# krea-ai/realtime-video

Measured on AMD Instinct MI355X. Metric: frames/sec at 832x480, 4-step 14B T2V (per-step DiT latency in config), higher is better.
Workload: dtype bf16

## Files before the change

### realtime_video_amd/csrc/gemm8.hip

```cpp
#include <atomic>
#include <mutex>
#include <type_traits>

#include "gemm_core.h"
#include "gemm_split.h"
#include "rtv_internal.h"

#ifndef RTV_G8_MFMA16
#define RTV_G8_MFMA16 1
#endif

namespace rtv {

namespace g8 {
constexpr int BM = 256, BN = 256, BK = 64;
constexpr int HALF_BYTES = 128 * BK * 2;
constexpr int A_OFF = 0;
constexpr int W_OFF = 6 * HALF_BYTES;
constexpr int LDS_BYTES = 10 * HALF_BYTES;
constexpr int THREADS = 512;
__device__ __forceinline__ int swz(int row, int chunk) { return chunk ^ ((row >> 1) & 7); }
}

#ifdef RTV_GEMM_TIMELINE
__device__ unsigned long long* g_timeline = nullptr;
#endif

__device__ __forceinline__ void g8_tile_mn(int tiles_m, int tiles_n, int tile_id, int* mt, int* nt) {
#if RTV_G8_BALANCED_GROUPS
  const int ngrp = (tiles_m + 7) >> 3;
  const int gq = tiles_m / ngrp, gr = tiles_m - gq * ngrp;
  const int big = (gq + 1) * tiles_n;
  int first_m, gm, in_group;
  if (tile_id < gr * big) {
    const int group = tile_id / big;
    gm = gq + 1;
    first_m = group * gm;
    in_group = tile_id - group * big;
  } else {
    const int t = tile_id - gr * big, sm = gq * tiles_n, group = t / sm;
    gm = gq;
    first_m = gr * (gq + 1) + group * gq;
    in_group = t - group * sm;
  }
#else
  constexpr int GROUP_M = 8;
  const int per_group = GROUP_M * tiles_n;
  const int group = tile_id / per_group;
  const int first_m = group * GROUP_M;
  const int gm = min(tiles_m - first_m, GROUP_M);
  const int in_group = tile_id - group * per_group;
#endif
  *mt = first_m + in_group % gm;
  *nt = in_group / gm;
}

template <bool F16>
__device__ __forceinline__ void gemm8m_body(const GemmParams& p, const SplitArgs& sp, int m0, int n0, int tile_id, int seg, int unit,
                                            int kt_begin, int kt_end, bool is_split);

template <bool F16, bool SKIP_IDLE>
__global__ __launch_bounds__(g8::THREADS, 2) void gemm8_kernel(GemmParams p, SplitArgs sp) {
  using namespace g8;
  int bid0 = blockIdx.x;
  if (sp.pair_units) {
    if (bid0 < sp.pair_pad) {
      if (bid0 >= sp.pair_units) return;
#pragma unroll 1
      for (int j = 0; j < 2; ++j) {
        const int tn = 2 * bid0 + j;
        if (tn >= p.tiles_n) break;
        if (j) __syncthreads();
        gemm8m_body<F16>(p, sp, sp.pair_m0, tn * BN, 0, 0, -1, 0, p.K / BK, false);
      }
      return;
    }
    bid0 -= sp.pair_pad;
  }
  if (sp.half_tail) {
    const int nhu = 2 * sp.tail_tiles;
    if (sp.split_first) bid0 = bid0 < nhu ? sp.first_unit + bid0 : bid0 - nhu;
    if (bid0 >= sp.first_unit) {
      const int v = xcd_remap(bid0 - sp.first_unit, nhu);
      const int tile_id = sp.first_unit + (v >> 1);
      int mt, nt;
      g8_tile_mn(p.tiles_m, p.tiles_n, tile_id, &mt, &nt);
      const int m0h = mt * BM + (v & 1) * 128;
      if (m0h >= p.M) return;
      gemm8m_body<F16>(p, sp, m0h, nt * BN, tile_id, 0, -1, 0, p.K / BK, false);
      return;
    }
    sp.S = 1;
    sp.split_first = 0;
  }
#ifdef RTV_GEMM_TIMELINE
  const unsigned long long tl_t0 = __builtin_amdgcn_s_memrealtime();
  const unsigned long long tl_c0 = __builtin_amdgcn_s_memtime();
  unsigned long long tl_t1 = 0;
#endif
  [[maybe_unused]] typedef TileCfg<256, 256, 64, 2, 4> Cfg;
  extern __shared__ __attribute__((aligned(16))) char smem[];

  const int tid = threadIdx.x;
  const int lane = tid & 63;
  const int wave = __builtin_amdgcn_readfirstlane(tid >> 6);
  const int wr = wave >> 2, wc = wave & 3;
  [[maybe_unused]] const int l31 = lane & 31, g = lane >> 5;

  const int nk_total = p.K / BK;
  int tile_id, seg, unit, kt_begin, kt_end;
  const bool is_split = split_unit_of_block(sp, bid0, nk_total, &tile_id, &unit, &seg, &kt_begin, &kt_end);
  int mt_, nt_;
  g8_tile_mn(p.tiles_m, p.tiles_n, tile_id, &mt_, &nt_);
  const int m0 = mt_ * BM;
  const int n0 = nt_ * BN;
  uint32_t src_off[4][2];
  {
    const int rsub = lane >> 3, cpos = lane & 7;
#pragma unroll
    for (int j = 0; j < 2; ++j) {
      const int row = j * 64 + wave * 8 + rsub;
      const int ch = swz(row, cpos) * 8;
#pragma unroll
      for (int h = 0; h < 2; ++h) {
        const int gm_row = min(m0 + h * 128 + row, p.M - 1);
        const int gn_row = min(n0 + h * 128 + row, p.N - 1);
        src_off[h][j] = ((uint32_t)gm_row * (uint32_t)p.lda + ch) * 2u;
        src_off[2 + h][j] = ((uint32_t)gn_row * (uint32_t)p.ldw + ch) * 2u;
      }
    }
  }
  __amdgpu_buffer_rsrc_t rsrcA = __builtin_amdgcn_make_buffer_rsrc((void*)p.A, 0, 0x7fffffff, 0x00020000);
  __amdgpu_buffer_rsrc_t rsrcW = __builtin_amdgcn_make_buffer_rsrc((void*)p.W, 0, 0x7fffffff, 0x00020000);
  auto stage_piece = [&](int kt, int a3, int h, int j, auto chk) {
    if (decltype(chk)::value && kt >= kt_end) return;
    const int slot = h < 2 ? A_OFF + (a3 * 2 + h) * HALF_BYTES : W_OFF + ((kt & 1) * 2 + (h - 2)) * HALF_BYTES;
    __builtin_amdgcn_raw_ptr_buffer_load_lds(h < 2 ? rsrcA : rsrcW, (RTV_LDS void*)(smem + slot + (j * 64 + wave * 8) * 128), 16,
                                             src_off[h][j], (unsigned)kt * (BK * 2), 0, 0);
  };

  const int b_row0 = (wc & 1) * 64;
#if RTV_G8_MFMA16
  const int l15 = lane & 15, q4 = lane >> 4;
  u32x4 af[4][2];
  u32x4 bfr[4][2];
  auto read_a = [&](int a3, int mq) {
    const char* s = smem + A_OFF + (a3 * 2 + wr) * HALF_BYTES;
#pragma unroll
    for (int mb = 0; mb < 4; ++mb) {
      const int row = mq * 64 + mb * 16 + l15;
#pragma unroll
      for (int ks = 0; ks < 2; ++ks) af[mb][ks] = *(const u32x4*)(s + row * 128 + (swz(row, ks * 4 + q4) << 4));
    }
  };
  auto read_w = [&](int wb) {
    const char* s = smem + W_OFF + (wb * 2 + (wc >> 1)) * HALF_BYTES;
#pragma unroll
    for (int nb = 0; nb < 4; ++nb) {
      const int row = b_row0 + nb * 16 + l15;
#pragma unroll
      for (int ks = 0; ks < 2; ++ks) bfr[nb][ks] = *(const u32x4*)(s + row * 128 + (swz(row, ks * 4 + q4) << 4));
    }
  };

  f32x4 acc[8][4];
#pragma unroll
  for (int mi = 0; mi < 8; ++mi)
#pragma unroll
    for (int ni = 0; ni < 4; ++ni)
#pragma unroll
      for (int r = 0; r < 4; ++r) acc[mi][ni][r] = 0.f;
#else
  u32x4 af[2][4];
  u32x4 bfr[2][4];
  auto read_a = [&](int a3, int mq) {
    const char* s = smem + A_OFF + (a3 * 2 + wr) * HALF_BYTES;
#pragma unroll
    for (int mb = 0; mb < 2; ++mb) {
      const int row = mq * 64 + mb * 32 + l31;
#pragma unroll
      for (int ks = 0; ks < 4; ++ks) af[mb][ks] = *(const u32x4*)(s + row * 128 + (swz(row, ks * 2 + g) << 4));
    }
  };
  auto read_w = [&](int wb) {
    const char* s = smem + W_OFF + (wb * 2 + (wc >> 1)) * HALF_BYTES;
#pragma unroll
    for (int nq = 0; nq < 2; ++nq) {
      const int row = b_row0 + nq * 32 + l31;
#pragma unroll
      for (int ks = 0; ks < 4; ++ks) bfr[nq][ks] = *(const u32x4*)(s + row * 128 + (swz(row, ks * 2 + g) << 4));
    }
  };

  f32x16 acc[4][2];
#pragma unroll
  for (int mi = 0; mi < 4; ++mi)
#pragma unroll
    for (int ni = 0; ni < 2; ++ni)
#pragma unroll
      for (int r = 0; r < 16; ++r) acc[mi][ni][r] = 0.f;
#endif

#define G8_FENCE() __builtin_amdgcn_sched_barrier(0)
#if RTV_G8_MFMA16
#define G8_STORE_LDS(...) store_tile_lds16<F16>(__VA_ARGS__)
#define G8_STORE_DIRECT(CFG, ...) store_tile16<F16>(__VA_ARGS__)
#else
#define G8_STORE_LDS(...) store_tile_lds<F16>(__VA_ARGS__)
#define G8_STORE_DIRECT(CFG, ...) store_tile<F16, CFG>(__VA_ARGS__)
#endif
#define G8_BARRIER()                  \
  do {                                \
    G8_FENCE();                       \
    __builtin_amdgcn_s_barrier();     \
    G8_FENCE();                       \
  } while (0)
#define G8_LDS_DONE()                                   \
  do {                                                  \
    asm volatile("s_waitcnt lgkmcnt(0)" ::: "memory");  \
    G8_FENCE();                                         \
  } while (0)

  const bool idle_rows = SKIP_IDLE && m0 + wr * 128 >= p.M;
  auto mma_half = [&](int mq, int st_kt, int st_a3, int h0, auto chk) {
    __builtin_amdgcn_s_setprio(1);
    int n = 0;
#if RTV_G8_MFMA16
#pragma unroll
    for (int ks = 0; ks < 2; ++ks)
#pragma unroll
      for (int nb = 0; nb < 4; ++nb)
#pragma unroll
        for (int mb = 0; mb < 4; ++mb) {
          acc[mq * 4 + mb][nb] = Mfma16<F16>::run(bfr[nb][ks], af[mb][ks], acc[mq * 4 + mb][nb]);
          ++n;
          if ((n & 7) == 4) {
            G8_FENCE();
            stage_piece(st_kt, st_a3, h0 + (n >> 4), (n >> 3) & 1, chk);
            G8_FENCE();
          }
        }
#else
#pragma unroll
    for (int ks = 0; ks < 4; ++ks)
#pragma unroll
      for (int nq = 0; nq < 2; ++nq)
#pragma unroll
        for (int mb = 0; mb < 2; ++mb) {
          acc[mq * 2 + mb][nq] = Mfma32<F16>::run(bfr[nq][ks], af[mb][ks], acc[mq * 2 + mb][nq]);
          ++n;
          if ((n & 3) == 2) {
            G8_FENCE();
            stage_piece(st_kt, st_a3, h0 + (n >> 3), (n >> 2) & 1, chk);
            G8_FENCE();
          }
        }
#endif
    __builtin_amdgcn_s_setprio(0);
  };

#pragma unroll
  for (int t = 0; t < 2; ++t)
#pragma unroll
    for (int hh = 0; hh < 4; ++hh) {
      const int h = (hh + 2) & 3;
      stage_piece(kt_begin + t, t, h, 0, std::true_type{});
      stage_piece(kt_begin + t, t, h, 1, std::true_type{});
    }
  if (kt_begin + 1 < kt_end) asm volatile("s_waitcnt vmcnt(8)" ::: "memory");
  else asm volatile("s_waitcnt vmcnt(0)" ::: "memory");
  G8_BARRIER();
  if (wr == 1) G8_BARRIER();

  int a3 = 0;
  auto k_tile = [&](const int kt, auto chk) {
    constexpr bool CHK = decltype(chk)::value;
    const int a3n = a3 == 0 ? 2 : a3 - 1;
    read_w(kt & 1);
    read_a(a3, 0);
    G8_LDS_DONE();
    G8_BARRIER();
    mma_half(0, kt + 2, a3n, 0, chk);
    G8_BARRIER();
    read_a(a3, 1);
    if (!CHK || kt + 2 < kt_end) asm volatile("s_waitcnt vmcnt(4)" ::: "memory");
    else asm volatile("s_waitcnt vmcnt(0)" ::: "memory");
    G8_LDS_DONE();
    G8_BARRIER();
    mma_half(1, kt + 2, a3n, 2, chk);
    G8_BARRIER();
    a3 = a3 == 2 ? 0 : a3 + 1;
  };
  auto idle_tile = [&](const int kt) {
    const int a3n = a3 == 0 ? 2 : a3 - 1;
    G8_BARRIER();
#pragma unroll
    for (int i = 0; i < 4; ++i) stage_piece(kt + 2, a3n, i >> 1, i & 1, std::true_type{});
    G8_BARRIER();
    if (kt + 2 < kt_end) asm volatile("s_waitcnt vmcnt(4)" ::: "memory");
    else asm volatile("s_waitcnt vmcnt(0)" ::: "memory");
    G8_BARRIER();
#pragma unroll
    for (int i = 0; i < 4; ++i) stage_piece(kt + 2, a3n, 2 + (i >> 1), i & 1, std::true_type{});
    G8_BARRIER();
    a3 = a3 == 2 ? 0 : a3 + 1;
  };
  int kt = kt_begin;
  if (idle_rows) {
    for (; kt < kt_end; ++kt) idle_tile(kt);
  } else {
    for (; kt + 2 < kt_end; ++kt) k_tile(kt, std::false_type{});
    for (; kt < kt_end; ++kt) k_tile(kt, std::true_type{});
  }
  if (wr == 0) G8_BARRIER();

#ifdef RTV_GEMM_TIMELINE
  tl_t1 = __builtin_amdgcn_s_memrealtime();
  const unsigned long long tl_c1 = __builtin_amdgcn_s_memtime();
  bool reducer = true;
  if (is_split) reducer = split_k_reduce(acc, sp, unit, seg, tile_id, smem, tid, wave, lane);
  if (!reducer) {
    if (g_timeline && tid == 0) {
      unsigned long long* t = g_timeline + (size_t)blockIdx.x * 4;
      t[0] = tl_t0;
      t[1] = tl_t1;
      t[2] = __builtin_amdgcn_s_memrealtime();
      t[3] = ((unsigned long long)(seg + 1) << 32) | (unsigned)tile_id;
    }
    return;
  }
#else
  if (is_split && !split_k_reduce(acc, sp, unit, seg, tile_id, smem, tid, wave, lane)) return;
#endif

  const bool wide = !((p.ldc | (p.residual ? p.ldr : 0)) & 7) && !(((uintptr_t)p.C | (uintptr_t)p.residual) & 15);
  if (wide) {
    if (is_split) __syncthreads();
#ifdef RTV_GEMM_TIMELINE
    unsigned long long tl_mid = 0;
    G8_STORE_LDS(p, m0 + wr * 128, n0 + wc * 64, lane, smem + wave * (128 * 128), acc, &tl_mid);
    if (g_timeline && tid == 0) g_timeline[(size_t)blockIdx.x * 4 + 1] = tl_mid | (1ull << 63);
    tl_t1 = tl_t1 ? tl_t1 : 0;
    if (g_timeline && tid == 0) {
      unsigned long long* t = g_timeline + (size_t)blockIdx.x * 4;
      t[0] = tl_t0;
      t[2] = __builtin_amdgcn_s_memrealtime();
      t[3] = ((unsigned long long)(is_split ? seg + 1 : 0) << 32) | (unsigned)tile_id;
      g_timeline[(size_t)(gridDim.x + blockIdx.x) * 4] = tl_t1;
      g_timeline[(size_t)(gridDim.x + blockIdx.x) * 4 + 1] = tl_c1 - tl_c0;
    }
    return;
#else
    G8_STORE_LDS(p, m0 + wr * 128, n0 + wc * 64, lane, smem + wave * (128 * 128), acc, nullptr);
#endif
  } else {
    G8_STORE_DIRECT(Cfg, p, m0 + wr * 128, n0 + wc * 64, lane, acc);
  }
#ifdef RTV_GEMM_TIMELINE
  if (g_timeline && tid == 0) {
    unsigned long long* t = g_timeline + (size_t)blockIdx.x * 4;
    t[0] = tl_t0;
    t[1] = tl_t1;
    t[2] = __builtin_amdgcn_s_memrealtime();
    t[3] = ((unsigned long long)(is_split ? seg + 1 : 0) << 32) | (unsigned)tile_id | (is_split ? 0x80000000u : 0u);
  }
#endif
}

static std::atomic<bool> g_gemm8_skip_idle{true};
static std::atomic<bool> g_gemm8_half_tail{true};
static std::atomic<bool> g_gemm8_ragged_strips{true};
namespace g8m {
constexpr int BM = 128, BN = 256, BK = 64;
constexpr int HALF_BYTES = 128 * BK * 2;
constexpr int LDS_BYTES = 9 * HALF_BYTES;
}

template <bool F16>
__device__ __forceinline__ void gemm8m_body(const GemmParams& p, const SplitArgs& sp, int m0, int n0, int tile_id, int seg, int unit,
                                            int kt_begin, int kt_end, bool is_split) {
  using namespace g8m;
  extern __shared__ __attribute__((aligned(16))) char smem[];
  const int tid = threadIdx.x;
  const int lane = tid & 63;
  const int wave = __builtin_amdgcn_readfirstlane(tid >> 6);
  const int wr = wave >> 2, wc = wave & 3;
  [[maybe_unused]] const int l31 = lane & 31, g = lane >> 5;

  uint32_t src_off[3][2];
  {
    const int rsub = lane >> 3, cpos = lane & 7;
#pragma unroll
    for (int j = 0; j < 2; ++j) {
      const int row = j * 64 + wave * 8 + rsub;
      const int ch = g8::swz(row, cpos) * 8;
      src_off[0][j] = ((uint32_t)min(m0 + row, p.M - 1) * (uint32_t)p.lda + ch) * 2u;
      src_off[1][j] = ((uint32_t)min(n0 + row, p.N - 1) * (uint32_t)p.ldw + ch) * 2u;
      src_off[2][j] = ((uint32_t)min(n0 + 128 + row, p.N - 1) * (uint32_t)p.ldw + ch) * 2u;
    }
  }
  __amdgpu_buffer_rsrc_t rsrcA = __builtin_amdgcn_make_buffer_rsrc((void*)p.A, 0, 0x7fffffff, 0x00020000);
  __amdgpu_buffer_rsrc_t rsrcW = __builtin_amdgcn_make_buffer_rsrc((void*)p.W, 0, 0x7fffffff, 0x00020000);
  auto stage_piece = [&](int kt, int b3, int h, int j, auto chk) {
    if (decltype(chk)::value && kt >= kt_end) return;
    __builtin_amdgcn_raw_ptr_buffer_load_lds(h == 0 ? rsrcA : rsrcW,
                                             (RTV_LDS void*)(smem + (b3 * 3 + h) * HALF_BYTES + (j * 64 + wave * 8) * 128), 16,
                                             src_off[h][j], (unsigned)kt * (BK * 2), 0, 0);
  };

#if RTV_G8_MFMA16
  const int l15 = lane & 15, q4 = lane >> 4;
  u32x4 af[4][2], bfr[4][2];
  auto read_frags = [&](int b3) {
    const char* sa = smem + (b3 * 3) * HALF_BYTES;
    const char* sw = smem + (b3 * 3 + 1 + (wc >> 1)) * HALF_BYTES;
#pragma unroll
    for (int nb = 0; nb < 4; ++nb) {
      const int row = (wc & 1) * 64 + nb * 16 + l15;
#pragma unroll
      for (int ks = 0; ks < 2; ++ks) bfr[nb][ks] = *(const u32x4*)(sw + row * 128 + (g8::swz(row, ks * 4 + q4) << 4));
    }
#pragma unroll
    for (int mb = 0; mb < 4; ++mb) {
      const int row = wr * 64 + mb * 16 + l15;
#pragma unroll
      for (int ks = 0; ks < 2; ++ks) af[mb][ks] = *(const u32x4*)(sa + row * 128 + (g8::swz(row, ks * 4 + q4) << 4));
    }
  };

  f32x4 acc[4][4];
#pragma unroll
  for (int mi = 0; mi < 4; ++mi)
#pragma unroll
    for (int ni = 0; ni < 4; ++ni)
#pragma unroll
      for (int r = 0; r < 4; ++r) acc[mi][ni][r] = 0.f;
#else
  u32x4 af[2][4], bfr[2][4];
  auto read_frags = [&](int b3) {
    const char* sa = smem + (b3 * 3) * HALF_BYTES;
    const char* sw = smem + (b3 * 3 + 1 + (wc >> 1)) * HALF_BYTES;
#pragma unroll
    for (int nq = 0; nq < 2; ++nq) {
      const int row = (wc & 1) * 64 + nq * 32 + l31;
#pragma unroll
      for (int ks = 0; ks < 4; ++ks) bfr[nq][ks] = *(const u32x4*)(sw + row * 128 + (g8::swz(row, ks * 2 + g) << 4));
    }
#pragma unroll
    for (int mb = 0; mb < 2; ++mb) {
      const int row = wr * 64 + mb * 32 + l31;
#pragma unroll
      for (int ks = 0; ks < 4; ++ks) af[mb][ks] = *(const u32x4*)(sa + row * 128 + (g8::swz(row, ks * 2 + g) << 4));
    }
  };

  f32x16 acc[2][2];
#pragma unroll
  for (int mi = 0; mi < 2; ++mi)
#pragma unroll
    for (int ni = 0; ni < 2; ++ni)
#pragma unroll
      for (int r = 0; r < 16; ++r) acc[mi][ni][r] = 0.f;
#endif

#pragma unroll
  for (int t = 0; t < 2; ++t)
#pragma unroll
    for (int h = 0; h < 3; ++h) {
      stage_piece(kt_begin + t, t, h, 0, std::true_type{});
      stage_piece(kt_begin + t, t, h, 1, std::true_type{});
    }
  if (wr == 1) {
#pragma unroll
    for (int h = 0; h < 3; ++h) {
      stage_piece(kt_begin + 2, 2, h, 0, std::true_type{});
      stage_piece(kt_begin + 2, 2, h, 1, std::true_type{});
    }
  }
  if (wr == 1) {
    if (kt_begin + 2 < kt_end) asm volatile("s_waitcnt vmcnt(6)" ::: "memory");
    else asm volatile("s_waitcnt vmcnt(0)" ::: "memory");
  } else {
    if (kt_begin + 1 < kt_end) asm volatile("s_waitcnt vmcnt(6)" ::: "memory");
    else asm volatile("s_waitcnt vmcnt(0)" ::: "memory");
  }
  G8_BARRIER();
  if (wr == 1) G8_BARRIER();

  int b3 = 0;
  auto k_tile = [&](const int kt, auto chk) {
    constexpr bool CHK = decltype(chk)::value;
    read_frags(b3);
    G8_LDS_DONE();
    G8_BARRIER();
    const int st_kt = kt + 2 + wr;
    const int st_b = wr ? b3 : (b3 == 0 ? 2 : b3 - 1);
    __builtin_amdgcn_s_setprio(1);
    int n = 0;
#if RTV_G8_MFMA16
#pragma unroll
    for (int ks = 0; ks < 2; ++ks)
#pragma unroll
      for (int nb = 0; nb < 4; ++nb)
#pragma unroll
        for (int mb = 0; mb < 4; ++mb) {
          acc[mb][nb] = Mfma16<F16>::run(bfr[nb][ks], af[mb][ks], acc[mb][nb]);
          ++n;
          if (n == 4 || n == 8 || n == 14 || n == 20 || n == 24 || n == 30) {
            const int pc = n == 4 ? 0 : n == 8 ? 1 : n == 14 ? 2 : n == 20 ? 3 : n == 24 ? 4 : 5;
            G8_FENCE();
            stage_piece(st_kt, st_b, pc >> 1, pc & 1, chk);
            G8_FENCE();
          }
        }
#else
#pragma unroll
    for (int ks = 0; ks < 4; ++ks)
#pragma unroll
      for (int nq = 0; nq < 2; ++nq)
#pragma unroll
        for (int mb = 0; mb < 2; ++mb) {
          acc[mb][nq] = Mfma32<F16>::run(bfr[nq][ks], af[mb][ks], acc[mb][nq]);
          ++n;
          if (n == 2 || n == 4 || n == 7 || n == 10 || n == 12 || n == 15) {
            const int pc = n == 2 ? 0 : n == 4 ? 1 : n == 7 ? 2 : n == 10 ? 3 : n == 12 ? 4 : 5;
            G8_FENCE();
            stage_piece(st_kt, st_b, pc >> 1, pc & 1, chk);
            G8_FENCE();
          }
        }
#endif
    __builtin_amdgcn_s_setprio(0);
    G8_FENCE();
    if (!CHK || st_kt < kt_end) asm volatile("s_waitcnt vmcnt(6)" ::: "memory");
    else asm volatile("s_waitcnt vmcnt(0)" ::: "memory");
    G8_BARRIER();
    b3 = b3 == 2 ? 0 : b3 + 1;
  };
  int kt = kt_begin;
  for (; kt + 3 < kt_end; ++kt) k_tile(kt, std::false_type{});
  for (; kt < kt_end; ++kt) k_tile(kt, std::true_type{});
  if (wr == 0) G8_BARRIER();

  if (is_split && !split_k_reduce(acc, sp, unit, seg, tile_id, smem, tid, wave, lane)) return;

  const bool wide = !((p.ldc | (p.residual ? p.ldr : 0)) & 7) && !(((uintptr_t)p.C | (uintptr_t)p.residual) & 15);
  if (wide) {
    if (is_split) __syncthreads();
    G8_STORE_LDS(p, m0 + wr * 64, n0 + wc * 64, lane, smem + wave * (64 * 128), acc, nullptr);
  } else {
    [[maybe_unused]] typedef TileCfg<128, 256, 64, 2, 4> CfgM;
    G8_STORE_DIRECT(CfgM, p, m0 + wr * 64, n0 + wc * 64, lane, acc);
  }
}

template <bool F16>
__global__ __launch_bounds__(g8::THREADS, 2) void gemm8m_kernel(GemmParams p, SplitArgs sp) {
  using namespace g8m;
  const int nk_total = p.K / BK;
  int tile_id, seg, unit, kt_begin, kt_end;
  const bool is_split = split_unit_of_block(sp, blockIdx.x, nk_total, &tile_id, &unit, &seg, &kt_begin, &kt_end);
  constexpr int GROUP_M = 8;
  const int per_group = GROUP_M * p.tiles_n;
  const int group = tile_id / per_group;
  const int first_m = group * GROUP_M;
  const int gm = min(p.tiles_m - first_m, GROUP_M);
  const int in_group = tile_id - group * per_group;
  gemm8m_body<F16>(p, sp, (first_m + in_group % gm) * BM, (in_group / gm) * BN, tile_id, seg, unit, kt_begin, kt_end, is_split);
}

struct SplitWorkspace {
  int device;
  hipStream_t stream;
  bool any_stream;
  float* slabs;
  int* counters;
};
constexpr int MAX_WORKSPACES = 64;
constexpr int MAX_DEVICES = 64;
static SplitWorkspace g_ws[MAX_WORKSPACES];
static int g_num_ws = 0;
static std::mutex g_ws_mu;

static int attach_workspace(bool any_stream, hipStream_t stream, void* ptr, size_t bytes) {
  int dev = 0;
  if (hipGetDevice(&dev) != hipSuccess) return set_error(-1, "gemm_set_workspace: cannot query the device");
  std::lock_guard<std::mutex> lk(g_ws_mu);
  int slot = -1;
  for (int i = 0; i < g_num_ws; ++i)
    if (g_ws[i].device == dev && g_ws[i].any_stream == any_stream && (any_stream || g_ws[i].stream == stream)) slot = i;
  if (!ptr) {
    if (slot >= 0) g_ws[slot] = g_ws[--g_num_ws];
    return 0;
  }
  if (((uintptr_t)ptr) & 255) return set_error(-1, "gemm_set_workspace: pointer must be 256-byte aligned");
  if (bytes < rtv_gemm_workspace_bytes()) return set_error(-1, "gemm_set_workspace: too small (rtv_gemm_workspace_bytes)");
  if (slot < 0) {
    if (g_num_ws == MAX_WORKSPACES) return set_error(-1, "gemm_set_workspace: too many workspaces attached");
    slot = g_num_ws++;
  }
  SplitWorkspace w{dev, stream, any_stream, (float*)ptr, (int*)((char*)ptr + (size_t)SPLIT_MAX_UNITS * SPLIT_SLAB_FLOATS * 4)};
  if (hipMemset(w.counters, 0, (size_t)SPLIT_MAX_UNITS * sizeof(int)) != hipSuccess) {
    if (slot == g_num_ws - 1) --g_num_ws;
    return set_error(-1, "gemm_set_workspace: cannot zero the arrival counters");
  }
  g_ws[slot] = w;
  return 0;
}

}

using namespace rtv;

#ifdef RTV_GEMM_TIMELINE
extern "C" int rtv_gemm_debug_timeline(unsigned long long* buf) {
  return hipMemcpyToSymbol(HIP_SYMBOL(g_timeline), &buf, sizeof(buf)) == hipSuccess ? 0 : -1;
}
#endif

extern "C" int rtv_gemm_set_half_tail(int on) {
  rtv::g_gemm8_half_tail.store(on != 0, std::memory_order_relaxed);
  return 0;
}

extern "C" int rtv_gemm_set_ragged_strips(int on) {
  rtv::g_gemm8_ragged_strips.store(on != 0, std::memory_order_relaxed);
  return 0;
}

extern "C" int rtv_gemm_set_skip_idle(int on) {
  rtv::g_gemm8_skip_idle.store(on != 0, std::memory_order_relaxed);
  return 0;
}

extern "C" size_t rtv_gemm_workspace_bytes(void) {
  return (size_t)SPLIT_MAX_UNITS * SPLIT_SLAB_FLOATS * 4 + (size_t)SPLIT_MAX_UNITS * 4 + 256;
}

extern "C" int rtv_gemm_set_workspace(void* ptr, size_t bytes) { return attach_workspace(true, nullptr, ptr, bytes); }

extern "C" int rtv_gemm_set_stream_workspace(rtv_stream_t stream, void* ptr, size_t bytes) {
  return attach_workspace(false, (hipStream_t)stream, ptr, bytes);
}

namespace rtv {

int plan_split_k(int T, int nk, bool allow_split, SplitArgs* sp, int* grid, hipStream_t stream, bool allow_half, int extra_units) {
  int dev = 0;
  if (hipGetDevice(&dev) != hipSuccess || dev < 0 || dev >= MAX_DEVICES) return set_error(-1, "gemm: cannot query the device");
  float* slabs = nullptr;
  int* counters = nullptr;
  const int G = device_num_cus();
  if (G <= 0) return set_error(-1, "gemm: cannot query the device");
  {
    std::lock_guard<std::mutex> lk(g_ws_mu);
    for (int i = 0; i < g_num_ws && allow_split; ++i) {
      const SplitWorkspace& w = g_ws[i];
      if (w.device != dev) continue;
      if (!w.any_stream && w.stream == stream) {
        slabs = w.slabs;
        counters = w.counters;
        break;
      }
      if (w.any_stream && !slabs) {
        slabs = w.slabs;
        counters = w.counters;
      }
    }
  }
  *sp = SplitArgs{T, 1, nullptr, nullptr, 0, 0, 0, 0, 0, 0};
  *grid = T;
  const int R = (T + extra_units) % G <= T ? (T + extra_units) % G : 0;
  if (allow_half && g_gemm8_half_tail.load(std::memory_order_relaxed) && R > 0 && T > R && G / R == 2 && nk <= 128) {
    sp->first_unit = T - R;
    sp->tail_tiles = R;
    sp->half_tail = 1;
    *grid = (T - R) + 2 * R;
    return 0;
  }
  if (allow_split && slabs && R > 0) {
    int S = G / R;
    if (S > 8) S = 8;
    if (S > nk / 4) S = nk / 4;
    if (S >= 2 && (size_t)R * S <= (size_t)SPLIT_MAX_UNITS) {
      sp->first_unit = T - R;
      sp->S = S;
      sp->slabs = slabs;
      sp->counters = counters;
      sp->tail_tiles = R;
      sp->split_first = (R * S * 4 <= G) ? 1 : 0;
      *grid = (T - R) + R * S;
    }
  }
  return 0;
}

template <bool F16, bool SKIP_IDLE>
static int launch_gemm8_t(GemmParams p, bool allow_split, hipStream_t stream) {
  p.tiles_m = (p.M + g8::BM - 1) / g8::BM;
  p.tiles_n = (p.N + g8::BN - 1) / g8::BN;
  auto kern = gemm8_kernel<F16, SKIP_IDLE>;
  static LdsAttr lds_attr;
  if (int st = ensure_dynamic_lds((const void*)kern, g8::LDS_BYTES, &lds_attr, "gemm8")) return st;
  SplitArgs sp;
  int grid = 0;
  const int G = device_num_cus();
  const int last_rows = p.M - (p.tiles_m - 1) * g8::BM;
  const int T0 = p.tiles_m * p.tiles_n;
  int pair_units = 0, pair_pad = 0;
  if (allow_split && g_gemm8_ragged_strips.load(std::memory_order_relaxed) && p.tiles_m >= 2 && last_rows <= 128 && G > 0 && T0 > G) {
    const int pu = (p.tiles_n + 1) / 2, pp = (pu + 7) & ~7;
    const int RA = T0 % G;
    if (RA > 0 && RA <= p.tiles_n - pp) {
      pair_units = pu;
      pair_pad = pp;
      p.tiles_m -= 1;
    }
  }
  if (int st = plan_split_k(p.tiles_m * p.tiles_n, p.K / g8::BK, allow_split, &sp, &grid, stream, true, pair_pad))
    return st;
  if (pair_units) {
    sp.pair_units = pair_units;
    sp.pair_pad = pair_pad;
    sp.pair_m0 = p.tiles_m * g8::BM;
    grid += pair_pad;
  }
  ProfScope prof(F16 ? PROF_CONV : PROF_GEMM, stream, 2.0 * p.M * (double)p.N * p.K);
  note_kernel(DK_GEMM8_256x256);
  hipLaunchKernelGGL(kern, dim3(grid), dim3(g8::THREADS), g8::LDS_BYTES, stream, p, sp);
  return check_launch("gemm8");
}

template <bool F16>
static int launch_gemm8m_t(GemmParams p, bool allow_split, hipStream_t stream) {
  p.tiles_m = (p.M + g8m::BM - 1) / g8m::BM;
  p.tiles_n = (p.N + g8m::BN - 1) / g8m::BN;
  auto kern = gemm8m_kernel<F16>;
  static LdsAttr lds_attr;
  if (int st = ensure_dynamic_lds((const void*)kern, g8m::LDS_BYTES, &lds_attr, "gemm8m")) return st;
  SplitArgs sp;
  int grid = 0;
  if (int st = plan_split_k(p.tiles_m * p.tiles_n, p.K / g8m::BK, allow_split, &sp, &grid, stream)) return st;
  ProfScope prof(F16 ? PROF_CONV : PROF_GEMM, stream, 2.0 * p.M * (double)p.N * p.K);
  note_kernel(DK_GEMM8M_128x256);
  hipLaunchKernelGGL(kern, dim3(grid), dim3(g8::THREADS), g8m::LDS_BYTES, stream, p, sp);
  return check_launch("gemm8m");
}

int launch_gemm8m(const GemmParams& p, bool f16, bool split, hipStream_t stream) {
  if ((size_t)p.M * p.lda * 2 > 0x7fffffffull || (size_t)p.N * p.ldw * 2 > 0x7fffffffull)
    return set_error(-1, "gemm8m: operand larger than 2 GiB");
  return f16 ? launch_gemm8m_t<true>(p, split, stream) : launch_gemm8m_t<false>(p, split, stream);
}

int launch_gemm8(const GemmParams& p, bool f16, bool split, hipStream_t stream) {
  if ((size_t)p.M * p.lda * 2 > 0x7fffffffull || (size_t)p.N * p.ldw * 2 > 0x7fffffffull)
    return set_error(-1, "gemm8: operand larger than 2 GiB");
  const int last_rows = p.M - (p.M - 1) / g8::BM * g8::BM;
  if (g_gemm8_skip_idle.load(std::memory_order_relaxed) && !f16 && last_rows <= 128) return launch_gemm8_t<false, true>(p, split, stream);
  return f16 ? launch_gemm8_t<true, false>(p, split, stream) : launch_gemm8_t<false, false>(p, split, stream);
}

}
```

Baseline: 18.74.

## Restructure GEMM global-to-LDS staging with immediate offsets, builtin waits, and loop-level priority

Reworks how the gemm8/gemm8m kernels issue buffer-to-LDS loads. Wave rows are laid out so the second piece's offset becomes an instruction immediate, with the resource base biased to compensate. LDS destination bases are precomputed in scalar registers, and the lgkmcnt wait uses the compiler builtin instead of inline asm. s_setprio moves from every MFMA burst to a loop-wide raise on the second wave row. The aim is to cut per-stage address arithmetic and scheduling overhead, but the bias shifts buffer bounds and the priority change alters wave arbitration. Optional modes that stage pieces before the barrier and timeline instrumentation are added but off by default.

```diff
diff --git a/realtime_video_amd/csrc/gemm8.hip b/realtime_video_amd/csrc/gemm8.hip
--- a/realtime_video_amd/csrc/gemm8.hip
+++ b/realtime_video_amd/csrc/gemm8.hip
@@ -9,6 +9,14 @@
 #ifndef RTV_G8_MFMA16
 #define RTV_G8_MFMA16 1
 #endif
+#ifndef RTV_G8_STAGE
+#define RTV_G8_STAGE 7
+#endif
+#define G8_ST_IMM ((RTV_G8_STAGE) & 1)
+#define G8_ST_WAIT ((RTV_G8_STAGE) & 2)
+#define G8_ST_PRIO ((RTV_G8_STAGE) & 4)
+#define G8_ST_YL (((RTV_G8_STAGE) & 8) ? (((RTV_G8_STAGE) & 32) ? 2 : 4) : 0)
+#define G8_ST_XL (((RTV_G8_STAGE) & 16) ? (((RTV_G8_STAGE) & 32) ? 2 : 4) : 0)
 
 namespace rtv {
 
@@ -19,11 +27,18 @@
 constexpr int W_OFF = 6 * HALF_BYTES;
 constexpr int LDS_BYTES = 10 * HALF_BYTES;
 constexpr int THREADS = 512;
+constexpr int W_ROWS = G8_ST_IMM ? 16 : 8, J_ROWS = G8_ST_IMM ? 8 : 64;
+constexpr int IMM_STEP = G8_ST_IMM ? J_ROWS * 128 : 0;
+constexpr int IMM_BIAS = IMM_STEP;
 __device__ __forceinline__ int swz(int row, int chunk) { return chunk ^ ((row >> 1) & 7); }
 }
 
 #ifdef RTV_GEMM_TIMELINE
 __device__ unsigned long long* g_timeline = nullptr;
+constexpr int TL_ROWS = 8192;
+__device__ __forceinline__ void timeline_grid() {
+  if (g_timeline && blockIdx.x == 0 && threadIdx.x == 0) g_timeline[(size_t)(TL_ROWS - 1) * 4] = gridDim.x;
+}
 #endif
 
 __device__ __forceinline__ void g8_tile_mn(int tiles_m, int tiles_n, int tile_id, int* mt, int* nt) {
@@ -63,6 +78,9 @@
 __global__ __launch_bounds__(g8::THREADS, 2) void gemm8_kernel(GemmParams p, SplitArgs sp) {
   using namespace g8;
   int bid0 = blockIdx.x;
+#ifdef RTV_GEMM_TIMELINE
+  timeline_grid();
+#endif
   if (sp.pair_units) {
     if (bid0 < sp.pair_pad) {
       if (bid0 >= sp.pair_units) return;
@@ -96,7 +114,7 @@
 #ifdef RTV_GEMM_TIMELINE
   const unsigned long long tl_t0 = __builtin_amdgcn_s_memrealtime();
   const unsigned long long tl_c0 = __builtin_amdgcn_s_memtime();
-  unsigned long long tl_t1 = 0;
+  unsigned long long tl_t1 = 0, tl_s0 = 0, tl_s1 = 0;
 #endif
   [[maybe_unused]] typedef TileCfg<256, 256, 64, 2, 4> Cfg;
   extern __shared__ __attribute__((aligned(16))) char smem[];
@@ -119,24 +137,32 @@
     const int rsub = lane >> 3, cpos = lane & 7;
 #pragma unroll
     for (int j = 0; j < 2; ++j) {
-      const int row = j * 64 + wave * 8 + rsub;
+      const int row = j * J_ROWS + wave * W_ROWS + rsub;
       const int ch = swz(row, cpos) * 8;
+      const uint32_t comp = (uint32_t)(IMM_BIAS - j * IMM_STEP);
 #pragma unroll
       for (int h = 0; h < 2; ++h) {
         const int gm_row = min(m0 + h * 128 + row, p.M - 1);
         const int gn_row = min(n0 + h * 128 + row, p.N - 1);
-        src_off[h][j] = ((uint32_t)gm_row * (uint32_t)p.lda + ch) * 2u;
-        src_off[2 + h][j] = ((uint32_t)gn_row * (uint32_t)p.ldw + ch) * 2u;
+        src_off[h][j] = ((uint32_t)gm_row * (uint32_t)p.lda + ch) * 2u + comp;
+        src_off[2 + h][j] = ((uint32_t)gn_row * (uint32_t)p.ldw + ch) * 2u + comp;
       }
     }
   }
-  __amdgpu_buffer_rsrc_t rsrcA = __builtin_amdgcn_make_buffer_rsrc((void*)p.A, 0, 0x7fffffff, 0x00020000);
-  __amdgpu_buffer_rsrc_t rsrcW = __builtin_amdgcn_make_buffer_rsrc((void*)p.W, 0, 0x7fffffff, 0x00020000);
+  __amdgpu_buffer_rsrc_t rsrcA = __builtin_amdgcn_make_buffer_rsrc((void*)((const char*)p.A - IMM_BIAS), 0, 0x7fffffff, 0x00020000);
+  __amdgpu_buffer_rsrc_t rsrcW = __builtin_amdgcn_make_buffer_rsrc((void*)((const char*)p.W - IMM_BIAS), 0, 0x7fffffff, 0x00020000);
+  const uint32_t lds_wave = (uint32_t)(uintptr_t)(RTV_LDS char*)smem + (uint32_t)wave * (W_ROWS * 128);
+  auto lds_op = [&](int kt, int a3, bool is_w) -> uint32_t {
+    return lds_wave + (is_w ? W_OFF + (kt & 1) * 2 * HALF_BYTES : A_OFF + a3 * 2 * HALF_BYTES);
+  };
+  auto stage_at = [&](int kt, uint32_t op, int h, int j, auto chk) {
+    if (decltype(chk)::value && kt >= kt_end) return;
+    RTV_LDS void* dst = (RTV_LDS void*)(uintptr_t)(op + (uint32_t)((h & 1) * HALF_BYTES + j * (J_ROWS * 128 - IMM_STEP)));
+    if (j) __builtin_amdgcn_raw_ptr_buffer_load_lds(h < 2 ? rsrcA : rsrcW, dst, 16, src_off[h][1], (unsigned)kt * (BK * 2), IMM_STEP, 0);
+    else __builtin_amdgcn_raw_ptr_buffer_load_lds(h < 2 ? rsrcA : rsrcW, dst, 16, src_off[h][0], (unsigned)kt * (BK * 2), 0, 0);
+  };
   auto stage_piece = [&](int kt, int a3, int h, int j, auto chk) {
-    if (decltype(chk)::value && kt >= kt_end) return;
-    const int slot = h < 2 ? A_OFF + (a3 * 2 + h) * HALF_BYTES : W_OFF + ((kt & 1) * 2 + (h - 2)) * HALF_BYTES;
-    __builtin_amdgcn_raw_ptr_buffer_load_lds(h < 2 ? rsrcA : rsrcW, (RTV_LDS void*)(smem + slot + (j * 64 + wave * 8) * 128), 16,
-                                             src_off[h][j], (unsigned)kt * (BK * 2), 0, 0);
+    stage_at(kt, lds_op(kt, a3, h >= 2), h, j, chk);
   };
 
   const int b_row0 = (wc & 1) * 64;
@@ -215,15 +241,37 @@
     __builtin_amdgcn_s_barrier();     \
     G8_FENCE();                       \
   } while (0)
-#define G8_LDS_DONE()                                   \
-  do {                                                  \
-    asm volatile("s_waitcnt lgkmcnt(0)" ::: "memory");  \
-    G8_FENCE();                                         \
+#if G8_ST_WAIT
+#define G8_LGKM0() __builtin_amdgcn_s_waitcnt(0xC07F)
+#else
+#define G8_LGKM0() asm volatile("s_waitcnt lgkmcnt(0)" ::: "memory")
+#endif
+#define G8_LDS_DONE() \
+  do {                \
+    G8_LGKM0();       \
+    G8_FENCE();       \
   } while (0)
+#if G8_ST_YL == 4
+#define G8_WAIT_Y() asm volatile("s_waitcnt vmcnt(8)" ::: "memory")
+#elif G8_ST_YL == 2
+#define G8_WAIT_Y() asm volatile("s_waitcnt vmcnt(6)" ::: "memory")
+#else
+#define G8_WAIT_Y() asm volatile("s_waitcnt vmcnt(4)" ::: "memory")
+#endif
+#if G8_ST_PRIO
+#define G8_PRIO(x) ((void)0)
+#define G8_PRIO_LOOP(wr, x)                          \
+  do {                                               \
+    if ((wr) == 1) __builtin_amdgcn_s_setprio(x);    \
+  } while (0)
+#else
+#define G8_PRIO(x) __builtin_amdgcn_s_setprio(x)
+#define G8_PRIO_LOOP(wr, x) ((void)0)
+#endif
 
   const bool idle_rows = SKIP_IDLE && m0 + wr * 128 >= p.M;
-  auto mma_half = [&](int mq, int st_kt, int st_a3, int h0, auto chk) {
-    __builtin_amdgcn_s_setprio(1);
+  auto mma_half = [&](int mq, int st_kt, uint32_t st_op, int h0, int first_piece, auto chk) {
+    G8_PRIO(1);
     int n = 0;
 #if RTV_G8_MFMA16
 #pragma unroll
@@ -234,9 +282,9 @@
         for (int mb = 0; mb < 4; ++mb) {
           acc[mq * 4 + mb][nb] = Mfma16<F16>::run(bfr[nb][ks], af[mb][ks], acc[mq * 4 + mb][nb]);
           ++n;
-          if ((n & 7) == 4) {
+          if ((n & 7) == 4 && (n >> 3) >= first_piece) {
             G8_FENCE();
-            stage_piece(st_kt, st_a3, h0 + (n >> 4), (n >> 3) & 1, chk);
+            stage_at(st_kt, st_op, h0 + (n >> 4), (n >> 3) & 1, chk);
             G8_FENCE();
           }
         }
@@ -249,14 +297,14 @@
         for (int mb = 0; mb < 2; ++mb) {
           acc[mq * 2 + mb][nq] = Mfma32<F16>::run(bfr[nq][ks], af[mb][ks], acc[mq * 2 + mb][nq]);
           ++n;
-          if ((n & 3) == 2) {
+          if ((n & 3) == 2 && (n >> 2) >= first_piece) {
             G8_FENCE();
-            stage_piece(st_kt, st_a3, h0 + (n >> 3), (n >> 2) & 1, chk);
+            stage_at(st_kt, st_op, h0 + (n >> 3), (n >> 2) & 1, chk);
             G8_FENCE();
           }
         }
 #endif
-    __builtin_amdgcn_s_setprio(0);
+    G8_PRIO(0);
   };
 
 #pragma unroll
@@ -271,37 +319,62 @@
   else asm volatile("s_waitcnt vmcnt(0)" ::: "memory");
   G8_BARRIER();
   if (wr == 1) G8_BARRIER();
-
+  G8_PRIO_LOOP(wr, 1);
+
+  auto early = [&](uint32_t op) {
+#if G8_ST_IMM
+    asm volatile("" : "+s"(op));
+#endif
+    return op;
+  };
   int a3 = 0;
   auto k_tile = [&](const int kt, auto chk) {
     constexpr bool CHK = decltype(chk)::value;
     const int a3n = a3 == 0 ? 2 : a3 - 1;
     read_w(kt & 1);
     read_a(a3, 0);
+    const uint32_t op_a = early(lds_op(kt + 2, a3n, false));
+#pragma unroll
+    for (int i = 0; i < G8_ST_XL; ++i) stage_at(kt + 2, op_a, i >> 1, i & 1, chk);
     G8_LDS_DONE();
     G8_BARRIER();
-    mma_half(0, kt + 2, a3n, 0, chk);
+#ifdef RTV_GEMM_TIMELINE_SEG
+    if (!CHK) tl_s0 = __builtin_amdgcn_s_memtime();
+    G8_FENCE();
+#endif
+    mma_half(0, kt + 2, op_a, 0, G8_ST_XL, chk);
+#ifdef RTV_GEMM_TIMELINE_SEG
+    G8_FENCE();
+    if (!CHK) tl_s1 = __builtin_amdgcn_s_memtime();
+#endif
     G8_BARRIER();
     read_a(a3, 1);
-    if (!CHK || kt + 2 < kt_end) asm volatile("s_waitcnt vmcnt(4)" ::: "memory");
+    const uint32_t op_w = early(lds_op(kt + 2, a3n, true));
+#pragma unroll
+    for (int i = 0; i < G8_ST_YL; ++i) stage_at(kt + 2, op_w, 2 + (i >> 1), i & 1, chk);
+    if (!CHK || kt + 2 < kt_end) G8_WAIT_Y();
     else asm volatile("s_waitcnt vmcnt(0)" ::: "memory");
     G8_LDS_DONE();
     G8_BARRIER();
-    mma_half(1, kt + 2, a3n, 2, chk);
+    mma_half(1, kt + 2, op_w, 2, G8_ST_YL, chk);
     G8_BARRIER();
     a3 = a3 == 2 ? 0 : a3 + 1;
   };
   auto idle_tile = [&](const int kt) {
     const int a3n = a3 == 0 ? 2 : a3 - 1;
-    G8_BARRIER();
-#pragma unroll
-    for (int i = 0; i < 4; ++i) stage_piece(kt + 2, a3n, i >> 1, i & 1, std::true_type{});
-    G8_BARRIER();
-    if (kt + 2 < kt_end) asm volatile("s_waitcnt vmcnt(4)" ::: "memory");
+#pragma unroll
+    for (int i = 0; i < G8_ST_XL; ++i) stage_piece(kt + 2, a3n, i >> 1, i & 1, std::true_type{});
+    G8_BARRIER();
+#pragma unroll
+    for (int i = G8_ST_XL; i < 4; ++i) stage_piece(kt + 2, a3n, i >> 1, i & 1, std::true_type{});
+    G8_BARRIER();
+#pragma unroll
+    for (int i = 0; i < G8_ST_YL; ++i) stage_piece(kt + 2, a3n, 2 + (i >> 1), i & 1, std::true_type{});
+    if (kt + 2 < kt_end) G8_WAIT_Y();
     else asm volatile("s_waitcnt vmcnt(0)" ::: "memory");
     G8_BARRIER();
 #pragma unroll
-    for (int i = 0; i < 4; ++i) stage_piece(kt + 2, a3n, 2 + (i >> 1), i & 1, std::true_type{});
+    for (int i = G8_ST_YL; i < 4; ++i) stage_piece(kt + 2, a3n, 2 + (i >> 1), i & 1, std::true_type{});
     G8_BARRIER();
     a3 = a3 == 2 ? 0 : a3 + 1;
   };
@@ -313,6 +386,7 @@
     for (; kt < kt_end; ++kt) k_tile(kt, std::true_type{});
   }
   if (wr == 0) G8_BARRIER();
+  G8_PRIO_LOOP(wr, 0);
 
 #ifdef RTV_GEMM_TIMELINE
   tl_t1 = __builtin_amdgcn_s_memrealtime();
@@ -348,6 +422,7 @@
       t[3] = ((unsigned long long)(is_split ? seg + 1 : 0) << 32) | (unsigned)tile_id;
       g_timeline[(size_t)(gridDim.x + blockIdx.x) * 4] = tl_t1;
       g_timeline[(size_t)(gridDim.x + blockIdx.x) * 4 + 1] = tl_c1 - tl_c0;
+      g_timeline[(size_t)(gridDim.x + blockIdx.x) * 4 + 2] = tl_s1 - tl_s0;
     }
     return;
 #else
@@ -380,6 +455,11 @@
 __device__ __forceinline__ void gemm8m_body(const GemmParams& p, const SplitArgs& sp, int m0, int n0, int tile_id, int seg, int unit,
                                             int kt_begin, int kt_end, bool is_split) {
   using namespace g8m;
+#ifdef RTV_GEMM_TIMELINE
+  const unsigned long long tl_t0 = __builtin_amdgcn_s_memrealtime();
+  const unsigned long long tl_c0 = __builtin_amdgcn_s_memtime();
+  unsigned long long tl_s0 = 0, tl_s1 = 0;
+#endif
   extern __shared__ __attribute__((aligned(16))) char smem[];
   const int tid = threadIdx.x;
   const int lane = tid & 63;
@@ -392,20 +472,25 @@
     const int rsub = lane >> 3, cpos = lane & 7;
 #pragma unroll
     for (int j = 0; j < 2; ++j) {
-      const int row = j * 64 + wave * 8 + rsub;
+      const int row = j * g8::J_ROWS + wave * g8::W_ROWS + rsub;
       const int ch = g8::swz(row, cpos) * 8;
-      src_off[0][j] = ((uint32_t)min(m0 + row, p.M - 1) * (uint32_t)p.lda + ch) * 2u;
-      src_off[1][j] = ((uint32_t)min(n0 + row, p.N - 1) * (uint32_t)p.ldw + ch) * 2u;
-      src_off[2][j] = ((uint32_t)min(n0 + 128 + row, p.N - 1) * (uint32_t)p.ldw + ch) * 2u;
-    }
-  }
-  __amdgpu_buffer_rsrc_t rsrcA = __builtin_amdgcn_make_buffer_rsrc((void*)p.A, 0, 0x7fffffff, 0x00020000);
-  __amdgpu_buffer_rsrc_t rsrcW = __builtin_amdgcn_make_buffer_rsrc((void*)p.W, 0, 0x7fffffff, 0x00020000);
+      const uint32_t comp = (uint32_t)(g8::IMM_BIAS - j * g8::IMM_STEP);
+      src_off[0][j] = ((uint32_t)min(m0 + row, p.M - 1) * (uint32_t)p.lda + ch) * 2u + comp;
+      src_off[1][j] = ((uint32_t)min(n0 + row, p.N - 1) * (uint32_t)p.ldw + ch) * 2u + comp;
+      src_off[2][j] = ((uint32_t)min(n0 + 128 + row, p.N - 1) * (uint32_t)p.ldw + ch) * 2u + comp;
+    }
+  }
+  __amdgpu_buffer_rsrc_t rsrcA = __builtin_amdgcn_make_buffer_rsrc((void*)((const char*)p.A - g8::IMM_BIAS), 0, 0x7fffffff, 0x00020000);
+  __amdgpu_buffer_rsrc_t rsrcW = __builtin_amdgcn_make_buffer_rsrc((void*)((const char*)p.W - g8::IMM_BIAS), 0, 0x7fffffff, 0x00020000);
+  const uint32_t lds_wave = (uint32_t)(uintptr_t)(RTV_LDS char*)smem + (uint32_t)wave * (g8::W_ROWS * 128);
+  auto stage_at = [&](int kt, uint32_t buf, int h, int j, auto chk) {
+    if (decltype(chk)::value && kt >= kt_end) return;
+    RTV_LDS void* dst = (RTV_LDS void*)(uintptr_t)(buf + (uint32_t)(h * HALF_BYTES + j * (g8::J_ROWS * 128 - g8::IMM_STEP)));
+    if (j) __builtin_amdgcn_raw_ptr_buffer_load_lds(h == 0 ? rsrcA : rsrcW, dst, 16, src_off[h][1], (unsigned)kt * (BK * 2), g8::IMM_STEP, 0);
+    else __builtin_amdgcn_raw_ptr_buffer_load_lds(h == 0 ? rsrcA : rsrcW, dst, 16, src_off[h][0], (unsigned)kt * (BK * 2), 0, 0);
+  };
   auto stage_piece = [&](int kt, int b3, int h, int j, auto chk) {
-    if (decltype(chk)::value && kt >= kt_end) return;
-    __builtin_amdgcn_raw_ptr_buffer_load_lds(h == 0 ? rsrcA : rsrcW,
-                                             (RTV_LDS void*)(smem + (b3 * 3 + h) * HALF_BYTES + (j * 64 + wave * 8) * 128), 16,
-                                             src_off[h][j], (unsigned)kt * (BK * 2), 0, 0);
+    stage_at(kt, lds_wave + (uint32_t)(b3 * 3 * HALF_BYTES), h, j, chk);
   };
 
 #if RTV_G8_MFMA16
@@ -486,16 +571,25 @@
   }
   G8_BARRIER();
   if (wr == 1) G8_BARRIER();
+  G8_PRIO_LOOP(wr, 1);
 
   int b3 = 0;
   auto k_tile = [&](const int kt, auto chk) {
     constexpr bool CHK = decltype(chk)::value;
     read_frags(b3);
-    G8_LDS_DONE();
-    G8_BARRIER();
     const int st_kt = kt + 2 + wr;
     const int st_b = wr ? b3 : (b3 == 0 ? 2 : b3 - 1);
-    __builtin_amdgcn_s_setprio(1);
+    uint32_t st_buf = lds_wave + (uint32_t)(st_b * 3 * HALF_BYTES);
+#if G8_ST_IMM
+    asm volatile("" : "+s"(st_buf));
+#endif
+    G8_LDS_DONE();
+    G8_BARRIER();
+#ifdef RTV_GEMM_TIMELINE_SEG
+    if (!CHK) tl_s0 = __builtin_amdgcn_s_memtime();
+    G8_FENCE();
+#endif
+    G8_PRIO(1);
     int n = 0;
 #if RTV_G8_MFMA16
 #pragma unroll
@@ -509,7 +603,7 @@
           if (n == 4 || n == 8 || n == 14 || n == 20 || n == 24 || n == 30) {
             const int pc = n == 4 ? 0 : n == 8 ? 1 : n == 14 ? 2 : n == 20 ? 3 : n == 24 ? 4 : 5;
             G8_FENCE();
-            stage_piece(st_kt, st_b, pc >> 1, pc & 1, chk);
+            stage_at(st_kt, st_buf, pc >> 1, pc & 1, chk);
             G8_FENCE();
           }
         }
@@ -525,13 +619,16 @@
           if (n == 2 || n == 4 || n == 7 || n == 10 || n == 12 || n == 15) {
             const int pc = n == 2 ? 0 : n == 4 ? 1 : n == 7 ? 2 : n == 10 ? 3 : n == 12 ? 4 : 5;
             G8_FENCE();
-            stage_piece(st_kt, st_b, pc >> 1, pc & 1, chk);
+            stage_at(st_kt, st_buf, pc >> 1, pc & 1, chk);
             G8_FENCE();
           }
         }
 #endif
-    __builtin_amdgcn_s_setprio(0);
+    G8_PRIO(0);
     G8_FENCE();
+#ifdef RTV_GEMM_TIMELINE_SEG
+    if (!CHK) tl_s1 = __builtin_amdgcn_s_memtime();
+#endif
     if (!CHK || st_kt < kt_end) asm volatile("s_waitcnt vmcnt(6)" ::: "memory");
     else asm volatile("s_waitcnt vmcnt(0)" ::: "memory");
     G8_BARRIER();
@@ -541,6 +638,26 @@
   for (; kt + 3 < kt_end; ++kt) k_tile(kt, std::false_type{});
   for (; kt < kt_end; ++kt) k_tile(kt, std::true_type{});
   if (wr == 0) G8_BARRIER();
+  G8_PRIO_LOOP(wr, 0);
+#ifdef RTV_GEMM_TIMELINE
+  if (g_timeline && tid == 0) {
+    const unsigned long long t1 = __builtin_amdgcn_s_memrealtime(), c1 = __builtin_amdgcn_s_memtime();
+    unsigned long long* t = g_timeline + (size_t)blockIdx.x * 4;
+    t[0] = tl_t0;
+    t[1] = t1;
+    t[3] = ((unsigned long long)(is_split ? seg + 1 : 0) << 32) | (unsigned)tile_id | (1ull << 62);
+    unsigned long long* u = g_timeline + (size_t)(gridDim.x + blockIdx.x) * 4;
+    u[0] = t1;
+    u[1] = c1 - tl_c0;
+    u[2] = tl_s1 - tl_s0;
+  }
+  struct TlEnd {
+    int tid;
+    __device__ ~TlEnd() {
+      if (g_timeline && tid == 0) g_timeline[(size_t)blockIdx.x * 4 + 2] = __builtin_amdgcn_s_memrealtime();
+    }
+  } tl_end{tid};
+#endif
 
   if (is_split && !split_k_reduce(acc, sp, unit, seg, tile_id, smem, tid, wave, lane)) return;
 
@@ -557,6 +674,9 @@
 template <bool F16>
 __global__ __launch_bounds__(g8::THREADS, 2) void gemm8m_kernel(GemmParams p, SplitArgs sp) {
   using namespace g8m;
+#ifdef RTV_GEMM_TIMELINE
+  timeline_grid();
+#endif
   const int nk_total = p.K / BK;
   int tile_id, seg, unit, kt_begin, kt_end;
   const bool is_split = split_unit_of_block(sp, blockIdx.x, nk_total, &tile_id, &unit, &seg, &kt_begin, &kt_end);
@@ -748,13 +868,13 @@
 }
 
 int launch_gemm8m(const GemmParams& p, bool f16, bool split, hipStream_t stream) {
-  if ((size_t)p.M * p.lda * 2 > 0x7fffffffull || (size_t)p.N * p.ldw * 2 > 0x7fffffffull)
+  if ((size_t)p.M * p.lda * 2 + g8::IMM_BIAS > 0x7fffffffull || (size_t)p.N * p.ldw * 2 + g8::IMM_BIAS > 0x7fffffffull)
     return set_error(-1, "gemm8m: operand larger than 2 GiB");
   return f16 ? launch_gemm8m_t<true>(p, split, stream) : launch_gemm8m_t<false>(p, split, stream);
 }
 
 int launch_gemm8(const GemmParams& p, bool f16, bool split, hipStream_t stream) {
-  if ((size_t)p.M * p.lda * 2 > 0x7fffffffull || (size_t)p.N * p.ldw * 2 > 0x7fffffffull)
+  if ((size_t)p.M * p.lda * 2 + g8::IMM_BIAS > 0x7fffffffull || (size_t)p.N * p.ldw * 2 + g8::IMM_BIAS > 0x7fffffffull)
     return set_error(-1, "gemm8: operand larger than 2 GiB");
   const int last_rows = p.M - (p.M - 1) / g8::BM * g8::BM;
   if (g_gemm8_skip_idle.load(std::memory_order_relaxed) && !f16 && last_rows <= 128) return launch_gemm8_t<false, true>(p, split, stream);
```

New measurement: 18.90, median of 6. No clear change (+0.8%).
